# google-research/nerf-from-image

Measured on NVIDIA H100. Metric: rays_per_sec_128x128_64+64spp, higher is better.
Workload: dtype f32

## Files before the change

### nerf_from_image_b200/csrc/nfi_forward_pipe.cuh

```cuda
#pragma once
#include <type_traits>

#include "nfi_forward.cuh"
#include "nfi_forward_tc.cuh"

namespace nfi {

#ifndef NFI_WAIT_NS
#define NFI_WAIT_NS 0
#endif
#define NFI_STEP_WAIT(bar, par) tc::mbar_wait_backoff<NFI_WAIT_NS>(bar, par)

__device__ __forceinline__ void mbar_arrive(uint64_t* bar) {
  asm volatile("mbarrier.arrive.shared::cta.b64 _, [%0];" ::"r"(tc::smem_u32(bar)) : "memory");
}

__device__ __forceinline__ float ld_relaxed(const float* p) {
  float v;
  asm volatile("ld.relaxed.cta.global.f32 %0, [%1];" : "=f"(v) : "l"(p) : "memory");
  return v;
}

__device__ __forceinline__ bool elect_one() {
  uint32_t pred;
  asm volatile(
      "{\n.reg .pred p;\nelect.sync _|p, 0xffffffff;\nselp.u32 %0, 1, 0, p;\n}\n"
      : "=r"(pred));
  return pred != 0;
}

struct TileCoord {
  int b, tile_x, tile_y;
};

__device__ __forceinline__ TileCoord tile_coord(int tile, int tiles_x, int tiles_y) {
  TileCoord c;
  const int per_img = tiles_x * tiles_y;
  c.b = tile / per_img;
  const int r = tile % per_img;
  const int bx = (tiles_x + 1) / 2;
  const int blk = r / 4, in = r % 4;
  int tx = 2 * (blk % bx) + (in & 1), ty = 2 * (blk / bx) + (in >> 1);
  if ((tiles_x & 1) || (tiles_y & 1)) {
    tx = r % tiles_x;
    ty = r / tiles_x;
  }
  c.tile_x = tx;
  c.tile_y = ty;
  return c;
}

constexpr int kPipeSlots = 3;
constexpr int kPipeStageBytes = 32768;
constexpr int kFwdStageBytes = 16384;
constexpr int kD2Ld = 20;
constexpr int kD2SlotBytes = kThreads * kD2Ld * 4;

__host__ __device__ inline size_t pipe_scratch_floats(int S, int nes) {
  return tc_scratch_floats_per_group(S) + (size_t)S * kThreads * nes;
}

constexpr int kViewTileBytes = kThreads * NFI_VIEW_FEATURES * 4;

template <int P, bool VD = false>
struct PipeCfg {
  static constexpr int kThreadsTotal = 256 + 128 * P;
  static constexpr int kStages = P + 1;
  static constexpr int kSmA = VD ? 41984 : 25600;
  static constexpr int kSmD2 = kSmA + kStages * kFwdStageBytes;
  static constexpr int kSmView = kSmD2 + kPipeSlots * kD2SlotBytes;
  static constexpr int kSmPal = kSmView + (VD ? kViewTileBytes : 0);
  static constexpr int kSmFrac = kSmPal + 48 * 4;
  static constexpr int kSmBars = kSmFrac + 128 * 4;
  static constexpr int kNumBars = 2 * kStages + 2 * kPipeSlots + 3;
  static constexpr int kSmBytes = kSmBars + kNumBars * 8;
  static constexpr int kActRegs = 136;
  static constexpr int kShadeRegs = 80;
  static constexpr int kProducerRegs = 88;
};

constexpr float kLog2e = 1.4426950408889634f;
constexpr float kLn2 = 0.6931471805599453f;
constexpr float kPadLogit = -1e30f;

__device__ __forceinline__ void decoder_layer2(const float (&d)[32], uint64_t w2_hi, uint64_t w2_lo,
                                               const float* __restrict__ b1, float* d2, int warp,
                                               int lane) {
  uint32_t hi[8][4], lo[8][4];
  tc::softplus_frag<true>(d, b1, lane & 3, hi, lo);
  float o[8];
#pragma unroll
  for (int i = 0; i < 8; ++i) o[i] = 0.f;
  tc::wgmma_fence();
  tc::layer2_mb(o, hi, lo, w2_hi, w2_lo);
  tc::wgmma_commit();
  tc::wgmma_wait<0>();
  tc::reg_fence(o);
  tc::store_frag_rows(o, d2, kD2Ld, warp, lane);
}

template <typename F>
__device__ __forceinline__ void decoder_step(uint64_t dsc_a, uint64_t w1_hi, uint64_t w1_lo,
                                             uint64_t w2_hi, uint64_t w2_lo,
                                             const float* __restrict__ b1, float* d2, int warp,
                                             int lane, F&& on_stage_read) {
#pragma unroll 1
  for (int mb = 0; mb < 2; ++mb) {
    float d[32];
#pragma unroll
    for (int i = 0; i < 32; ++i) d[i] = 0.f;
    tc::wgmma_fence();
    tc::layer1_mb(d, dsc_a + mb * (8192 >> 4), dsc_a + ((16384 + mb * 8192) >> 4), w1_hi, w1_lo);
    tc::wgmma_commit();
    tc::wgmma_wait<0>();
    tc::reg_fence(d);
    if (mb == 1) on_stage_read();
    decoder_layer2(d, w2_hi, w2_lo, b1, d2 + 64 * mb * kD2Ld, warp, lane);
  }
}

template <typename F>
__device__ __forceinline__ void decoder_step_fp32(const unsigned char* stage, uint64_t w1_hi,
                                                  uint64_t w1_lo, uint64_t w2_hi, uint64_t w2_lo,
                                                  const float* __restrict__ b1, float* d2, int warp,
                                                  int lane, F&& on_stage_read) {
  float fa[4][4], fb[4][4];
  tc::load_afrag_sw128(fa, stage, 0, warp, lane);
  tc::load_afrag_sw128(fb, stage, 64, warp, lane);
  on_stage_read();
#pragma unroll 1
  for (int mb = 0; mb < 2; ++mb) {
    uint32_t a_hi[4][4], a_lo[4][4];
#pragma unroll
    for (int kb = 0; kb < 4; ++kb)
#pragma unroll
      for (int s = 0; s < 4; ++s) tc::put_split(a_hi, a_lo, kb, s, fa[kb][s]);
    float d[32];
#pragma unroll
    for (int i = 0; i < 32; ++i) d[i] = 0.f;
    tc::wgmma_fence();
    tc::layer1_mb_rs(d, a_hi, a_lo, w1_hi, w1_lo);
    tc::wgmma_commit();
    tc::wgmma_wait<0>();
    tc::reg_fence(d);
    decoder_layer2(d, w2_hi, w2_lo, b1, d2 + 64 * mb * kD2Ld, warp, lane);
#pragma unroll
    for (int kb = 0; kb < 4; ++kb)
#pragma unroll
      for (int s = 0; s < 4; ++s) fa[kb][s] = fb[kb][s];
  }
}

__device__ __forceinline__ void fill_view_tile(const nfi_render_params& p, const TileCoord& tcd,
                                               const float* __restrict__ b2f, float4* vt, int wig,
                                               int lane) {
  const int g = lane >> 2, t = lane & 3;
#pragma unroll
// ... 286 lines not shown
  const float* noise_t;
  const float* noise_u;
  const float* frac;
  int S, wig;
  bool explicit_noise;
};
template <int N>
__device__ __forceinline__ void resample_rows_impl(const ResampleArgs& a, int first, int count,
                                                   float tnear, float tfar, size_t ray, bool valid,
                                                   int lane) {
  const int S = a.S;
  if (count <= 0) return;
  struct In {
    LaneVec<N> w, n, u;
    size_t rayj;
  };
  auto load = [&](int j, In& in) {
    in.rayj = ((size_t)__shfl_sync(kFull, (unsigned)(ray >> 32), j) << 32) |
              (size_t)__shfl_sync(kFull, (unsigned)ray, j);
    const int col = 32 * a.wig + j;
#pragma unroll
    for (int i = 0; i < N; ++i) {
      const int e = 32 * i + lane;
      in.w.v[i] = (e < S) ? ldcg(a.sc_w + e * kThreads + col) : 0.f;
      in.n.v[i] = 0.f;
      if (a.explicit_noise) {
        in.n.v[i] = (e < S) ? a.noise_t[in.rayj * S + e] : 0.f;
        in.u.v[i] = (e < S) ? a.noise_u[in.rayj * S + e] : 2.f;
      } else {
        in.u.v[i] = (e < S) ? linspace01(e, S) : 2.f;
      }
    }
  };
  In cur, nxt;
  load(first, cur);
#pragma unroll 1
  for (int j = first; j < first + count; ++j) {
    load(j + 1 < first + count ? j + 1 : j, nxt);
    const float nearj = __shfl_sync(kFull, tnear, j), farj = __shfl_sync(kFull, tfar, j);
    const bool validj = __shfl_sync(kFull, (int)valid, j) != 0;
    const int col = 32 * a.wig + j;
    const float spanj = farj - nearj;
    LaneVec<N> t;
#pragma unroll
    for (int i = 0; i < N; ++i)
      t.v[i] = lerp_torch(nearj, farj, a.frac[32 * i + lane]) + cur.n.v[i] * (spanj / (float)S);
    const LaneVec<N> z = resample_ray<N>(cur.w, t, cur.u, !a.explicit_noise, S, lane);
#pragma unroll
    for (int i = 0; i < N; ++i) {
      const int e = 32 * i + lane;
      if (e < S) a.sc_zf[e * kThreads + col] = z.v[i];
      if (a.z_fine != nullptr && validj && e < S) a.z_fine[cur.rayj * S + e] = z.v[i];
    }
    cur = nxt;
  }
}
template <int NOUT_PAD, int EXTRA, bool FINE, int P, bool DBG, int NSLOT = 2, bool VD = false>
__global__ void __launch_bounds__(PipeCfg<P>::kThreadsTotal, 1)
render_forward_pipe(const nfi_render_params p, const unsigned char* __restrict__ wimg,
                    float* __restrict__ scratch) {
  using Cfg = PipeCfg<P, VD>;
  static_assert(!(VD && DBG), "the phase timers are not instantiated for the view-conditioned kernel");
  constexpr int kImgBytes = VD ? kVdBytes : kWiBytes;
  constexpr int kImgB1 = VD ? kVdB1 : kWiB1, kImgB2 = VD ? kVdHead : kWiB2;
  constexpr int NA_ = NOUT_PAD - 1;
  constexpr int NE = (EXTRA == 1) ? 3 : (EXTRA == 2 ? NA_ : 0);
  constexpr int NES = (EXTRA == 2) ? NA_ : 0;
  extern __shared__ __align__(1024) unsigned char smem_raw[];
  unsigned char* base = smem_raw;
  const int tid = threadIdx.x, lane = tid & 31;
  const int hw_wg = __shfl_sync(kFull, tid >> 7, 0);
  const int wg = (hw_wg < P) ? hw_wg + 3 : (P + 1 - hw_wg);
  const int gt = tid & 127;
  const int wig = __shfl_sync(kFull, gt >> 5, 0);
  const int S = p.num_samples;

  uint64_t* bars = reinterpret_cast<uint64_t*>(base + Cfg::kSmBars);
  constexpr int NS = Cfg::kStages;
  uint64_t* full = bars;
  uint64_t* a_free = full + NS;
  uint64_t* d2_full = a_free + NS;
  uint64_t* slot_free = d2_full + kPipeSlots;
  uint64_t* cw_ready = slot_free + kPipeSlots;
  uint64_t* zf_ready = cw_ready + 1;
  uint64_t* wbar = zf_ready + 1;
  float* d2s = reinterpret_cast<float*>(base + Cfg::kSmD2);
  const float* b1s = reinterpret_cast<const float*>(base + kImgB1);
  const float* b2s = reinterpret_cast<const float*>(base + kImgB2);
  float* pal = reinterpret_cast<float*>(base + Cfg::kSmPal);
  float* frac = reinterpret_cast<float*>(base + Cfg::kSmFrac);
  if (tid < 128) frac[tid] = (float)tid / (float)S;

  if (tid == 0) {
    if (tc::smem_u32(base) & 1023u) __trap();
    for (int i = 0; i < NS; ++i) {
      tc::mbar_init(&full[i], kWarps);
      tc::mbar_init(&a_free[i], kWarps);
    }
    for (int i = 0; i < kPipeSlots; ++i) {
      tc::mbar_init(&d2_full[i], kWarps);
      tc::mbar_init(&slot_free[i], kWarps);
    }
    tc::mbar_init(cw_ready, kWarps);
    tc::mbar_init(zf_ready, (2 + P) * kWarps);
    tc::mbar_init(wbar, 1);
    tc::fence_mbar_init();
  }
  __syncthreads();
  if (tid == 0) {
    tc::mbar_expect_tx(wbar, kImgBytes);
    tc::tma_bulk_g2s(base, wimg, kImgBytes, wbar);
  }
  tc::mbar_wait(wbar, 0);

  const int tiles_x = (p.width + kTileW - 1) / kTileW;
  const int tiles_y = (p.height + kTileH - 1) / kTileH;
  const int n_tiles = tiles_x * tiles_y * p.batch;
  const int my_tiles =
      ((int)blockIdx.x < n_tiles) ? (n_tiles - 1 - (int)blockIdx.x) / (int)gridDim.x + 1 : 0;
  const uint32_t total_steps = (uint32_t)my_tiles * (uint32_t)S * (FINE ? 2u : 1u);
  const int R = p.plane_res;
  const float inv_range = 1.f / p.scene_range;
  const bool explicit_noise = (p.noise_mode == NFI_NOISE_EXPLICIT);
  const bool dbg_skip_gather = (p.mlp_mode & 0x100) != 0;
  const bool dbg_skip_consumer = (p.mlp_mode & 0x200) != 0;
  const bool dbg_window = (p.mlp_mode & 0x800) != 0;
  const bool dbg_time = DBG && (p.mlp_mode & 0x1000) && p.normals != nullptr && blockIdx.x == 0 &&
                        lane == 0 && (wg <= 3) && wg != 2 && wig == 0;
  long long tacc[DBG ? 10 : 1];
  long long tprev = 0;
  if (DBG)
    for (int i = 0; i < 10; ++i) tacc[i] = 0;
#define NFI_T(i)                         \
  if (DBG && dbg_time) {                 \
    const long long now__ = clock64();   \
    tacc[i] += now__ - tprev;            \
    tprev = now__;                       \
  }
  float* slab = scratch + (size_t)blockIdx.x * pipe_scratch_floats(S, NES);
  float4* sc_srgb = reinterpret_cast<float4*>(slab);
  float* sc_t = slab + (size_t)4 * S * kThreads;
  float* sc_w = sc_t + (size_t)S * kThreads;
  float* sc_zf = sc_w + (size_t)S * kThreads;
  float* sc_e = sc_zf + (size_t)S * kThreads;

  constexpr int kRsParts = 2 + P;
  auto rs_first = [](int part) {
    constexpr int base_rows = 32 / kRsParts, rem = 32 % kRsParts;
    return part * base_rows + min(max(part - 2, 0), rem);
  };
  auto resample_rows = [&](int part, float tnear, float tfar, size_t ray, bool valid) {
    const int first = rs_first(part), count = rs_first(part + 1) - first;
    ResampleArgs ra;
    ra.sc_w = sc_w;
    ra.sc_zf = sc_zf;
    ra.z_fine = p.z_fine;
    ra.noise_t = p.noise_t;
    ra.noise_u = p.noise_u;
    ra.frac = frac;
    ra.S = S;
    ra.wig = wig;
    ra.explicit_noise = explicit_noise;
    resample_rows_impl<NSLOT>(ra, first, count, tnear, tfar, ray, valid, lane);
  };

  if (wg >= 3) {
    asm volatile("setmaxnreg.dec.sync.aligned.u32 %0;" ::"n"(Cfg::kProducerRegs));
    const int set = wg - 3;
    uint32_t n = 0;
    uint32_t tile_it = 0;
    for (int tile = blockIdx.x; tile < n_tiles; tile += gridDim.x, ++tile_it) {
      const TileCoord tcd = tile_coord(tile, tiles_x, tiles_y);
      const int b = tcd.b;
      int px, py;
      tile_pixel(tcd.tile_x, tcd.tile_y, wig, lane, px, py);
      const bool valid = (px < p.width) && (py < p.height);
      px = min(px, p.width - 1);
      py = min(py, p.height - 1);
      const size_t ray = ((size_t)b * p.height + py) * p.width + px;
      Ray r;
      setup_ray(p, b, py, px, r);
      const float span = r.tfar - r.tnear;
      const uint32_t plane_bytes = (uint32_t)R * (uint32_t)R * 128u;
      const unsigned char* planes_b =
          reinterpret_cast<const unsigned char*>(p.planes) + (size_t)b * 3 * plane_bytes;
      for (int pass = 0; pass < (FINE ? 2 : 1); ++pass) {
        if (pass == 1) {
          tc::mbar_wait(cw_ready, tile_it & 1);
          resample_rows(2 + set, r.tnear, r.tfar, ray, valid);
          __threadfence_block();
          __syncwarp();
          if (lane == 0) mbar_arrive(zf_ready);
          tc::mbar_wait(zf_ready, tile_it & 1);
        }
        int s = (int)(((uint32_t)set + (uint32_t)P - (n % P)) % P);
        auto fetch = [&](int ss) -> float {
          if (ss >= S) return 0.f;
          if (pass == 0) return explicit_noise ? p.noise_t[ray * S + ss] : 0.f;
          return ld_relaxed(sc_zf + ss * kThreads + gt);
        };
        float nxt = fetch(s);
        for (; s < S; s += P) {
          const uint32_t st = (n + (uint32_t)s) % NS, u = (n + (uint32_t)s) / NS;
          unsigned char* const stage = base + Cfg::kSmA + st * kFwdStageBytes;
          const float cur = nxt;
          nxt = fetch(s + P);
          if (DBG && dbg_time) tprev = clock64();
          NFI_STEP_WAIT(&a_free[st], (u & 1) ^ 1);
          NFI_T(0)
          float t;
          if (pass == 0)
            t = lerp_torch(r.tnear, r.tfar, frac[s]) + cur * (span / (float)S);
          else
            t = cur;
          const float x0 = (r.ox + r.dx * t) * inv_range, x1 = (r.oy + r.dy * t) * inv_range,
                      x2 = (r.oz + r.dz * t) * inv_range;
          ByteTaps tp;
          byte_taps(x0, x1, R, 0u, tp.o[0], tp.fx[0], tp.fy[0]);
          byte_taps(x0, x2, R, plane_bytes >> 4, tp.o[1], tp.fx[1], tp.fy[1]);
          byte_taps(x1, x2, R, plane_bytes >> 3, tp.o[2], tp.fx[2], tp.fy[2]);
          NFI_T(1)
          if (dbg_window) {
            tp.o[0] &= 0x7FFu;
            tp.o[1] &= 0x7FFu;
            tp.o[2] &= 0x7FFu;
          }
          if (!dbg_skip_gather)
            gather_to_tiles_lean<TileStore::kFp32>(planes_b, R, tp, stage, nullptr, 32 * wig, lane);
          NFI_T(2)
          __syncwarp();
          if (lane == 0) mbar_arrive(&full[st]);
          NFI_T(3)
          if (DBG && dbg_time) tacc[9] += 1;
        }
        n += (uint32_t)S;
      }
    }
    if (DBG && dbg_time)
      for (int i = 0; i < 10; ++i) p.normals[i] = (float)tacc[i];
  } else if (wg == 0) {
    asm volatile("setmaxnreg.inc.sync.aligned.u32 %0;" ::"n"(Cfg::kActRegs));
    const uint32_t base_s = tc::smem_u32(base);
    const uint64_t dsc_w1_hi = tc::gmma_desc_sw128(base_s + kWiW1Hi);
    const uint64_t dsc_w1_lo = tc::gmma_desc_sw128(base_s + kWiW1Lo);
    const uint64_t dsc_w2_hi = tc::gmma_desc_sw128(base_s + (VD ? kVdW2Hi : kWiW2Hi));
    const uint64_t dsc_w2_lo = tc::gmma_desc_sw128(base_s + (VD ? kVdW2Lo : kWiW2Lo));
    const float4* vt = reinterpret_cast<const float4*>(base + Cfg::kSmView) + gt;
    uint32_t st = 0, u = 0, sl = 0, v = 0;
    auto activate = [&]() {
      if (DBG && dbg_time && tprev == 0) tprev = clock64();
      NFI_T(2)
      NFI_STEP_WAIT(&full[st], u & 1);
      NFI_STEP_WAIT(&slot_free[sl], (v & 1) ^ 1);
      NFI_T(0)
      float* d2 = d2s + sl * (kThreads * kD2Ld);
      if constexpr (VD) {
        decoder_step_vd(base + Cfg::kSmA + st * kFwdStageBytes, dsc_w1_hi, dsc_w1_lo, dsc_w2_hi,
                        dsc_w2_lo, tc::gmma_desc_sw128(base_s + kVdW3Hi),
                        tc::gmma_desc_sw128(base_s + kVdW3Lo), b1s, vt, d2, wig, lane, [&]() {
                          __syncwarp();
                          if (lane == 0) mbar_arrive(&a_free[st]);
                        });
      } else if (!dbg_skip_consumer) {
        decoder_step_fp32(base + Cfg::kSmA + st * kFwdStageBytes, dsc_w1_hi, dsc_w1_lo, dsc_w2_hi,
                          dsc_w2_lo, b1s, d2, wig, lane, [&]() {
                            __syncwarp();
                            if (lane == 0) mbar_arrive(&a_free[st]);
                          });
      } else {
        __syncwarp();
        if (lane == 0) mbar_arrive(&a_free[st]);
      }
      __syncwarp();
      if (lane == 0) mbar_arrive(&d2_full[sl]);
      if (++st == NS) { st = 0; ++u; }
      if (++sl == kPipeSlots) { sl = 0; ++v; }
      NFI_T(1)
      if (DBG && dbg_time) tacc[9] += 1;
    };
    uint32_t tile_it = 0;
    for (int tile = blockIdx.x; tile < n_tiles; tile += gridDim.x, ++tile_it) {
      if constexpr (VD)
        fill_view_tile(p, tile_coord(tile, tiles_x, tiles_y),
                       reinterpret_cast<const float*>(base + kVdB2f),
                       reinterpret_cast<float4*>(base + Cfg::kSmView) + gt, wig, lane);
      for (int s = 0; s < S; ++s) activate();
      if (FINE) {
        const TileCoord tcd = tile_coord(tile, tiles_x, tiles_y);
        int px, py;
        tile_pixel(tcd.tile_x, tcd.tile_y, wig, lane, px, py);
        const bool valid = (px < p.width) && (py < p.height);
        px = min(px, p.width - 1);
        py = min(py, p.height - 1);
        const size_t ray = ((size_t)tcd.b * p.height + py) * p.width + px;
        Ray r;
        setup_ray(p, tcd.b, py, px, r);
        tc::mbar_wait(cw_ready, tile_it & 1);
        NFI_T(3)
        resample_rows(1, r.tnear, r.tfar, ray, valid);
        __threadfence_block();
        __syncwarp();
        if (lane == 0) mbar_arrive(zf_ready);
        NFI_T(4)
        for (int s = 0; s < S; ++s) activate();
      }
    }
    if (DBG && dbg_time)
      for (int i = 0; i < 10; ++i) p.normals[16 + i] = (float)tacc[i];
  } else {
    asm volatile("setmaxnreg.dec.sync.aligned.u32 %0;" ::"n"(Cfg::kShadeRegs));
    uint32_t sl = 0, v = 0;
    FieldConst fc;
    fc.A = p.n_attention;
    fc.use_sdf = p.use_sdf;
    fc.inv_beta = p.use_sdf ? 1.f / p.beta[0] : 0.f;
    fc.inv_alpha = p.use_sdf ? 1.f / p.alpha[0] : 0.f;

    uint32_t tile_it = 0;
    for (int tile = blockIdx.x; tile < n_tiles; tile += gridDim.x, ++tile_it) {
      const TileCoord tcd = tile_coord(tile, tiles_x, tiles_y);
      const int b = tcd.b;
      int px, py;
      tile_pixel(tcd.tile_x, tcd.tile_y, wig, lane, px, py);
      const bool valid = (px < p.width) && (py < p.height);
      px = min(px, p.width - 1);
      py = min(py, p.height - 1);
      const size_t ray = ((size_t)b * p.height + py) * p.width + px;
      Ray r;
      setup_ray(p, b, py, px, r);
      const float span = r.tfar - r.tnear;

      tc::bar_sync(1, kThreads);
      if (gt < 48)
        pal[gt] = (p.n_attention > 0 && gt < p.n_attention * 3)
                      ? p.palette[(size_t)b * p.n_attention * 3 + gt]
                      : 0.f;
      tc::bar_sync(1, kThreads);
      Compositor<NE, true> comp;
      comp.init();

      auto shade = [&](float t, float& sigma, float& cr, float& cg, float& cb, float* ex) {
        const float* d2 = d2s + sl * (kThreads * kD2Ld) + gt * kD2Ld;
        if (DBG && dbg_time && tprev == 0) tprev = clock64();
        NFI_T(2)
        NFI_STEP_WAIT(&d2_full[sl], v & 1);
        NFI_T(0)
        float o16[16];
#pragma unroll
        for (int o4 = 0; o4 < 4; ++o4) {
          const float4 x = *reinterpret_cast<const float4*>(d2 + 4 * o4);
          o16[4 * o4] = x.x;
          o16[4 * o4 + 1] = x.y;
          o16[4 * o4 + 2] = x.z;
          o16[4 * o4 + 3] = x.w;
        }
        __syncwarp();
        if (lane == 0) mbar_arrive(&slot_free[sl]);
        if (++sl == kPipeSlots) { sl = 0; ++v; }
        const float wx = r.ox + r.dx * t, wy = r.oy + r.dy * t, wz = r.oz + r.dz * t;
        const float x0 = wx * inv_range, x1 = wy * inv_range, x2 = wz * inv_range;
        const float keep =
            (fabsf(x0) > 1.f || fabsf(x1) > 1.f || fabsf(x2) > 1.f) ? 0.f : 1.f;
        float out[NOUT_PAD];
#pragma unroll
        for (int o4 = 0; o4 < NOUT_PAD / 4; ++o4) {
          const float4 bb = *reinterpret_cast<const float4*>(b2s + 4 * o4);
          out[4 * o4] = o16[4 * o4] + bb.x;
          out[4 * o4 + 1] = o16[4 * o4 + 1] + bb.y;
          out[4 * o4 + 2] = o16[4 * o4 + 2] + bb.z;
          out[4 * o4 + 3] = o16[4 * o4 + 3] + bb.w;
        }
        if (dbg_skip_consumer) {
          sigma = out[0];
          cr = cg = cb = out[1];
        } else {
          field_head_fast<NOUT_PAD>(out, fc, pal, keep, sigma, cr, cg, cb,
                                    EXTRA == 2 ? ex : nullptr);
        }
        if (EXTRA == 1) {
          ex[0] = wx;
          ex[1] = wy;
          ex[2] = wz;
        }
        NFI_T(1)
        if (DBG && dbg_time) tacc[9] += 1;
      };

      {
        float wT = 1.f, prev_t = 0.f, prev_s = 0.f;
        const float4* nz4 = reinterpret_cast<const float4*>(p.noise_t + ray * S);
        const float4 zero4 = make_float4(0.f, 0.f, 0.f, 0.f);
        float4 nzc = explicit_noise ? nz4[0] : zero4;
        float4 nzn = (explicit_noise && S > 4) ? nz4[1] : zero4;
        const float jit = span / (float)S;
        for (int s = 0; s < S; ++s) {
          const int sq = s & 3;
          const float nz = sq == 0 ? nzc.x : (sq == 1 ? nzc.y : (sq == 2 ? nzc.z : nzc.w));
          const float t = lerp_torch(r.tnear, r.tfar, frac[s]) + nz * jit;
          if (sq == 3) {
            nzc = nzn;
            nzn = (explicit_noise && s + 5 < S) ? nz4[(s + 5) >> 2] : zero4;
          }
          float sigma, cr, cg, cb;
          float ex[NE > 0 ? NE : 1];
          shade(t, sigma, cr, cg, cb, ex);
          if (FINE) {
            sc_srgb[s * kThreads + gt] = make_float4(sigma, cr, cg, cb);
            sc_t[s * kThreads + gt] = t;
#pragma unroll
            for (int a = 0; a < NES; ++a) sc_e[((size_t)s * NES + a) * kThreads + gt] = ex[a];
            if (s > 0) {
              const float delta = (t - prev_t) * r.dn;
              const float a = 1.f - __expf(-prev_s * delta);
              sc_w[(s - 1) * kThreads + gt] = a * wT;
              wT = wT * ((1.f - a) + 1e-10f);
            }
            prev_t = t;
            prev_s = sigma;
          } else {
            comp.push(t, sigma, cr, cg, cb, ex, r.dn);
          }
          NFI_T(3)
        }
      }

      if (FINE) {
        sc_w[(S - 1) * kThreads + gt] = 0.f;
        __threadfence_block();
        __syncwarp();
        if (lane == 0) mbar_arrive(cw_ready);
        tc::mbar_wait(cw_ready, tile_it & 1);
        NFI_T(4)
        resample_rows(0, r.tnear, r.tfar, ray, valid);
        __threadfence_block();
        __syncwarp();
        if (lane == 0) mbar_arrive(zf_ready);
        tc::mbar_wait(zf_ready, tile_it & 1);
        NFI_T(5)

        int c = 0;
        float ct0 = ldcg(sc_t + gt), ct1 = ldcg(sc_t + kThreads + gt);
        float4 cq0 = __ldcg(sc_srgb + gt), cq1 = __ldcg(sc_srgb + kThreads + gt);
        auto take_coarse = [&]() {
          float ce[NE > 0 ? NE : 1];
          if (EXTRA == 1) {
            ce[0] = r.ox + r.dx * ct0;
            ce[1] = r.oy + r.dy * ct0;
            ce[2] = r.oz + r.dz * ct0;
          }
#pragma unroll
          for (int a = 0; a < NES; ++a) ce[a] = ldcg(sc_e + ((size_t)c * NES + a) * kThreads + gt);
          comp.push(ct0, cq0.x, cq0.y, cq0.z, cq0.w, ce, r.dn);
          ++c;
          ct0 = ct1;
          cq0 = cq1;
          if (c + 1 < S) {
            ct1 = ldcg(sc_t + (c + 1) * kThreads + gt);
            cq1 = __ldcg(sc_srgb + (c + 1) * kThreads + gt);
          }
        };
        float z0 = ldcg(sc_zf + gt);
        float z1 = (S > 1) ? ldcg(sc_zf + kThreads + gt) : 0.f;
        for (int k = 0; k < S; ++k) {
          const float z = z0;
          z0 = z1;
          z1 = (k + 2 < S) ? ldcg(sc_zf + (k + 2) * kThreads + gt) : 0.f;
          float sigma, cr, cg, cb;
          float ex[NE > 0 ? NE : 1];
          shade(z, sigma, cr, cg, cb, ex);
          while (c < S && ct0 <= z) take_coarse();
          comp.push(z, sigma, cr, cg, cb, ex, r.dn);
          NFI_T(3)
        }
        while (c < S) take_coarse();
        NFI_T(6)
      }

      if (valid) {
        float bg = 0.f;
        if (p.white_background) bg = 1.f - comp.am;
        p.rgb[ray * 3 + 0] = comp.ar + bg;
        p.rgb[ray * 3 + 1] = comp.ag + bg;
        p.rgb[ray * 3 + 2] = comp.ab + bg;
        p.depth[ray] = comp.ad;
        p.mask[ray] = comp.am;
        for (int q = 0; q < p.n_peers; ++q) {
          float* pr = p.peer_rgb[q] + ray * 3;
          pr[0] = comp.ar + bg;
          pr[1] = comp.ag + bg;
          pr[2] = comp.ab + bg;
          p.peer_depth[q][ray] = comp.ad;
          p.peer_mask[q][ray] = comp.am;
        }
        if (EXTRA == 1 && p.extra != nullptr)
          for (int a = 0; a < 3; ++a) p.extra[ray * 3 + a] = comp.ae[a];
        if (EXTRA == 2 && p.extra != nullptr)
          for (int a = 0; a < NE; ++a)
            if (a < p.n_attention) p.extra[ray * p.n_attention + a] = comp.ae[a];
      }
    }
    if (DBG && dbg_time)
      for (int i = 0; i < 10; ++i) p.normals[32 + i] = (float)tacc[i];
  }
#undef NFI_T
  __syncthreads();
  if (p.n_peers > 0 && p.peer_done != nullptr && tid == 0) {
    __threadfence_system();
    const unsigned done = atomicAdd(p.peer_done, 1u);
    if (done == gridDim.x - 1) {
      __threadfence();
      *p.peer_done = 0u;
      for (int q = 0; q < p.n_peers; ++q)
        asm volatile("st.release.sys.global.u32 [%0], %1;" ::"l"(p.peer_signal[q]), "r"(p.peer_epoch)
                     : "memory");
      const long long t0 = clock64();
      for (int q = 0; q < p.n_peers; ++q) {
        const uint32_t* flag = p.peer_signal_self + p.peer_rank[q];
        uint32_t v;
        do {
          asm volatile("ld.acquire.sys.global.u32 %0, [%1];" : "=r"(v) : "l"(flag) : "memory");
          if ((int)(v - p.peer_epoch) >= 0) break;
          __nanosleep(200);
          if (clock64() - t0 > 60000000000LL) __trap();
        } while (true);
      }
    }
  }
}

}
```

Before: 35.97 million.

## Software-pipeline coarse and fine passes across tiles with double-buffered scratch

```diff
diff --git a/nerf_from_image_b200/csrc/nfi_forward_pipe.cuh b/nerf_from_image_b200/csrc/nfi_forward_pipe.cuh
--- a/nerf_from_image_b200/csrc/nfi_forward_pipe.cuh
+++ b/nerf_from_image_b200/csrc/nfi_forward_pipe.cuh
@@ -13,6 +13,17 @@
 
 __device__ __forceinline__ void mbar_arrive(uint64_t* bar) {
   asm volatile("mbarrier.arrive.shared::cta.b64 _, [%0];" ::"r"(tc::smem_u32(bar)) : "memory");
+}
+
+__device__ __forceinline__ bool mbar_test_wait(uint64_t* bar, uint32_t parity) {
+  uint32_t ok;
+  asm volatile(
+      "{\n.reg .pred p;\nmbarrier.test_wait.parity.shared::cta.b64 p, [%1], %2;\n"
+      "selp.u32 %0, 1, 0, p;\n}\n"
+      : "=r"(ok)
+      : "r"(tc::smem_u32(bar)), "r"(parity)
+      : "memory");
+  return ok != 0;
 }
 
 __device__ __forceinline__ float ld_relaxed(const float* p) {
@@ -56,8 +67,11 @@
 constexpr int kD2Ld = 20;
 constexpr int kD2SlotBytes = kThreads * kD2Ld * 4;
 
+__host__ __device__ inline size_t pipe_scratch_slot_floats(int S, int nes) {
+  return tc_scratch_floats_per_group(S) + (size_t)S * kThreads * nes;
+}
 __host__ __device__ inline size_t pipe_scratch_floats(int S, int nes) {
-  return tc_scratch_floats_per_group(S) + (size_t)S * kThreads * nes;
+  return 2 * pipe_scratch_slot_floats(S, nes);
 }
 
 constexpr int kViewTileBytes = kThreads * NFI_VIEW_FEATURES * 4;
@@ -70,9 +84,9 @@
   static constexpr int kSmD2 = kSmA + kStages * kFwdStageBytes;
   static constexpr int kSmView = kSmD2 + kPipeSlots * kD2SlotBytes;
   static constexpr int kSmPal = kSmView + (VD ? kViewTileBytes : 0);
-  static constexpr int kSmFrac = kSmPal + 48 * 4;
+  static constexpr int kSmFrac = kSmPal + 2 * 48 * 4;
   static constexpr int kSmBars = kSmFrac + 128 * 4;
-  static constexpr int kNumBars = 2 * kStages + 2 * kPipeSlots + 3;
+  static constexpr int kNumBars = 2 * kStages + 2 * kPipeSlots + 5;
   static constexpr int kSmBytes = kSmBars + kNumBars * 8;
   static constexpr int kActRegs = 136;
   static constexpr int kShadeRegs = 80;
@@ -525,8 +539,8 @@
   uint64_t* d2_full = a_free + NS;
   uint64_t* slot_free = d2_full + kPipeSlots;
   uint64_t* cw_ready = slot_free + kPipeSlots;
-  uint64_t* zf_ready = cw_ready + 1;
-  uint64_t* wbar = zf_ready + 1;
+  uint64_t* zf_ready = cw_ready + 2;
+  uint64_t* wbar = zf_ready + 2;
   float* d2s = reinterpret_cast<float*>(base + Cfg::kSmD2);
   const float* b1s = reinterpret_cast<const float*>(base + kImgB1);
   const float* b2s = reinterpret_cast<const float*>(base + kImgB2);
@@ -544,8 +558,10 @@
       tc::mbar_init(&d2_full[i], kWarps);
       tc::mbar_init(&slot_free[i], kWarps);
     }
-    tc::mbar_init(cw_ready, kWarps);
-    tc::mbar_init(zf_ready, (2 + P) * kWarps);
+    for (int i = 0; i < 2; ++i) {
+      tc::mbar_init(&cw_ready[i], kWarps);
+      tc::mbar_init(&zf_ready[i], P * kWarps);
+    }
     tc::mbar_init(wbar, 1);
     tc::fence_mbar_init();
   }
@@ -561,7 +577,6 @@
   const int n_tiles = tiles_x * tiles_y * p.batch;
   const int my_tiles =
       ((int)blockIdx.x < n_tiles) ? (n_tiles - 1 - (int)blockIdx.x) / (int)gridDim.x + 1 : 0;
-  const uint32_t total_steps = (uint32_t)my_tiles * (uint32_t)S * (FINE ? 2u : 1u);
   const int R = p.plane_res;
   const float inv_range = 1.f / p.scene_range;
   const bool explicit_noise = (p.noise_mode == NFI_NOISE_EXPLICIT);
@@ -570,33 +585,64 @@
   const bool dbg_window = (p.mlp_mode & 0x800) != 0;
   const bool dbg_time = DBG && (p.mlp_mode & 0x1000) && p.normals != nullptr && blockIdx.x == 0 &&
                         lane == 0 && (wg <= 3) && wg != 2 && wig == 0;
-  long long tacc[DBG ? 10 : 1];
+  constexpr int kNT = DBG ? 12 : 1;
+  long long tacc[kNT];
   long long tprev = 0;
   if (DBG)
-    for (int i = 0; i < 10; ++i) tacc[i] = 0;
+    for (int i = 0; i < kNT; ++i) tacc[i] = 0;
 #define NFI_T(i)                         \
   if (DBG && dbg_time) {                 \
     const long long now__ = clock64();   \
     tacc[i] += now__ - tprev;            \
     tprev = now__;                       \
   }
-  float* slab = scratch + (size_t)blockIdx.x * pipe_scratch_floats(S, NES);
-  float4* sc_srgb = reinterpret_cast<float4*>(slab);
-  float* sc_t = slab + (size_t)4 * S * kThreads;
-  float* sc_w = sc_t + (size_t)S * kThreads;
-  float* sc_zf = sc_w + (size_t)S * kThreads;
-  float* sc_e = sc_zf + (size_t)S * kThreads;
-
-  constexpr int kRsParts = 2 + P;
-  auto rs_first = [](int part) {
-    constexpr int base_rows = 32 / kRsParts, rem = 32 % kRsParts;
-    return part * base_rows + min(max(part - 2, 0), rem);
+  struct Slot {
+    float4* srgb;
+    float* t;
+    float* w;
+    float* zf;
+    float* e;
   };
-  auto resample_rows = [&](int part, float tnear, float tfar, size_t ray, bool valid) {
-    const int first = rs_first(part), count = rs_first(part + 1) - first;
+  auto slot_of = [&](int k) {
+    float* slab = scratch + (size_t)blockIdx.x * pipe_scratch_floats(S, NES) +
+                  (size_t)(k & 1) * pipe_scratch_slot_floats(S, NES);
+    Slot o;
+    o.srgb = reinterpret_cast<float4*>(slab);
+    o.t = slab + (size_t)4 * S * kThreads;
+    o.w = o.t + (size_t)S * kThreads;
+    o.zf = o.w + (size_t)S * kThreads;
+    o.e = o.zf + (size_t)S * kThreads;
+    return o;
+  };
+  struct RowRay {
+    int b;
+    bool valid;
+    size_t ray;
+    Ray r;
+  };
+  auto row_ray = [&](int k) {
+    const TileCoord tcd = tile_coord((int)blockIdx.x + k * (int)gridDim.x, tiles_x, tiles_y);
+    int px, py;
+    tile_pixel(tcd.tile_x, tcd.tile_y, wig, lane, px, py);
+    RowRay o;
+    o.b = tcd.b;
+    o.valid = (px < p.width) && (py < p.height);
+    px = min(px, p.width - 1);
+    py = min(py, p.height - 1);
+    o.ray = ((size_t)tcd.b * p.height + py) * p.width + px;
+    setup_ray(p, tcd.b, py, px, o.r);
+    return o;
+  };
+
+  auto rs_first = [](int set) {
+    constexpr int base_rows = 32 / P, rem = 32 % P;
+    return set * base_rows + min(set, rem);
+  };
+  auto resample_rows = [&](int k, int first, int count, const RowRay& rr) {
+    const Slot sc = slot_of(k);
     ResampleArgs ra;
-    ra.sc_w = sc_w;
-    ra.sc_zf = sc_zf;
+    ra.sc_w = sc.w;
+    ra.sc_zf = sc.zf;
     ra.z_fine = p.z_fine;
     ra.noise_t = p.noise_t;
     ra.noise_u = p.noise_u;
@@ -604,83 +650,109 @@
     ra.S = S;
     ra.wig = wig;
     ra.explicit_noise = explicit_noise;
-    resample_rows_impl<NSLOT>(ra, first, count, tnear, tfar, ray, valid, lane);
+    resample_rows_impl<NSLOT>(ra, first, count, rr.r.tnear, rr.r.tfar, rr.ray, rr.valid, lane);
   };
 
   if (wg >= 3) {
     asm volatile("setmaxnreg.dec.sync.aligned.u32 %0;" ::"n"(Cfg::kProducerRegs));
     const int set = wg - 3;
+    const int rs0 = rs_first(set), rs_n = rs_first(set + 1) - rs0;
     uint32_t n = 0;
-    uint32_t tile_it = 0;
-    for (int tile = blockIdx.x; tile < n_tiles; tile += gridDim.x, ++tile_it) {
-      const TileCoord tcd = tile_coord(tile, tiles_x, tiles_y);
-      const int b = tcd.b;
-      int px, py;
-      tile_pixel(tcd.tile_x, tcd.tile_y, wig, lane, px, py);
-      const bool valid = (px < p.width) && (py < p.height);
-      px = min(px, p.width - 1);
-      py = min(py, p.height - 1);
-      const size_t ray = ((size_t)b * p.height + py) * p.width + px;
-      Ray r;
-      setup_ray(p, b, py, px, r);
+    auto resample_rest = [&](int k, int done, const RowRay& rq) {
+      if (done < rs_n) {
+        tc::mbar_wait(&cw_ready[k & 1], (k >> 1) & 1);
+        resample_rows(k, rs0 + done, rs_n - done, rq);
+      }
+      __threadfence_block();
+      __syncwarp();
+      if (lane == 0) mbar_arrive(&zf_ready[k & 1]);
+    };
+    auto run_pass = [&](int k, bool fine_pass, int rs) {
+      const RowRay rr = row_ray(k);
+      const Slot sc = slot_of(k);
+      const Ray& r = rr.r;
       const float span = r.tfar - r.tnear;
       const uint32_t plane_bytes = (uint32_t)R * (uint32_t)R * 128u;
       const unsigned char* planes_b =
-          reinterpret_cast<const unsigned char*>(p.planes) + (size_t)b * 3 * plane_bytes;
-      for (int pass = 0; pass < (FINE ? 2 : 1); ++pass) {
-        if (pass == 1) {
-          tc::mbar_wait(cw_ready, tile_it & 1);
-          resample_rows(2 + set, r.tnear, r.tfar, ray, valid);
-          __threadfence_block();
-          __syncwarp();
-          if (lane == 0) mbar_arrive(zf_ready);
-          tc::mbar_wait(zf_ready, tile_it & 1);
+          reinterpret_cast<const unsigned char*>(p.planes) + (size_t)rr.b * 3 * plane_bytes;
+      if (fine_pass) {
+        if (DBG && dbg_time) tprev = clock64();
+        tc::mbar_wait(&zf_ready[k & 1], (k >> 1) & 1);
+        NFI_T(5)
+      }
+      RowRay rq;
+      if (rs >= 0) rq = row_ray(rs);
+      int s = (int)(((uint32_t)set + (uint32_t)P - (n % P)) % P);
+      const int n_own = (S - s + P - 1) / P;
+      int j = 0, done = 0;
+      bool cw_seen = false;
+      auto fetch = [&](int ss) -> float {
+        if (ss >= S) return 0.f;
+        if (!fine_pass) return explicit_noise ? p.noise_t[rr.ray * S + ss] : 0.f;
+        return ld_relaxed(sc.zf + ss * kThreads + gt);
+      };
+      float nxt = fetch(s);
+      for (; s < S; s += P, ++j) {
+        const uint32_t st = (n + (uint32_t)s) % NS, u = (n + (uint32_t)s) / NS;
+        unsigned char* const stage = base + Cfg::kSmA + st * kFwdStageBytes;
+        const float cur = nxt;
+        nxt = fetch(s + P);
+        if (DBG && dbg_time) tprev = clock64();
+        NFI_STEP_WAIT(&a_free[st], (u & 1) ^ 1);
+        NFI_T(0)
+        float t;
+        if (!fine_pass)
+          t = lerp_torch(r.tnear, r.tfar, frac[s]) + cur * (span / (float)S);
+        else
+          t = cur;
+        const float x0 = (r.ox + r.dx * t) * inv_range, x1 = (r.oy + r.dy * t) * inv_range,
+                    x2 = (r.oz + r.dz * t) * inv_range;
+        ByteTaps tp;
+        byte_taps(x0, x1, R, 0u, tp.o[0], tp.fx[0], tp.fy[0]);
+        byte_taps(x0, x2, R, plane_bytes >> 4, tp.o[1], tp.fx[1], tp.fy[1]);
+        byte_taps(x1, x2, R, plane_bytes >> 3, tp.o[2], tp.fx[2], tp.fy[2]);
+        NFI_T(1)
+        if (dbg_window) {
+          tp.o[0] &= 0x7FFu;
+          tp.o[1] &= 0x7FFu;
+          tp.o[2] &= 0x7FFu;
         }
-        int s = (int)(((uint32_t)set + (uint32_t)P - (n % P)) % P);
-        auto fetch = [&](int ss) -> float {
-          if (ss >= S) return 0.f;
-          if (pass == 0) return explicit_noise ? p.noise_t[ray * S + ss] : 0.f;
-          return ld_relaxed(sc_zf + ss * kThreads + gt);
-        };
-        float nxt = fetch(s);
-        for (; s < S; s += P) {
-          const uint32_t st = (n + (uint32_t)s) % NS, u = (n + (uint32_t)s) / NS;
-          unsigned char* const stage = base + Cfg::kSmA + st * kFwdStageBytes;
-          const float cur = nxt;
-          nxt = fetch(s + P);
+        if (!dbg_skip_gather)
+          gather_to_tiles_lean<TileStore::kFp32>(planes_b, R, tp, stage, nullptr, 32 * wig, lane);
+        NFI_T(2)
+        __syncwarp();
+        if (lane == 0) mbar_arrive(&full[st]);
+        NFI_T(3)
+        if (rs >= 0) {
+          const int upto = (rs_n * (j + 1) + n_own - 1) / n_own;
+          if (upto > done && !cw_seen)
+            cw_seen = __all_sync(kFull, mbar_test_wait(&cw_ready[rs & 1], (rs >> 1) & 1));
+          if (upto > done && cw_seen) {
+            resample_rows(rs, rs0 + done, upto - done, rq);
+            done = upto;
+          }
+          NFI_T(4)
+        }
+        if (DBG && dbg_time) tacc[9] += 1;
+      }
+      n += (uint32_t)S;
+      if (rs >= 0) resample_rest(rs, done, rq);
+    };
+    for (int k = 0; k <= my_tiles; ++k) {
+      if (k < my_tiles) run_pass(k, false, (FINE && k >= 1) ? k - 1 : -1);
+      if (FINE && k >= 1) {
+        if (k == my_tiles) {
           if (DBG && dbg_time) tprev = clock64();
-          NFI_STEP_WAIT(&a_free[st], (u & 1) ^ 1);
-          NFI_T(0)
-          float t;
-          if (pass == 0)
-            t = lerp_torch(r.tnear, r.tfar, frac[s]) + cur * (span / (float)S);
-          else
-            t = cur;
-          const float x0 = (r.ox + r.dx * t) * inv_range, x1 = (r.oy + r.dy * t) * inv_range,
-                      x2 = (r.oz + r.dz * t) * inv_range;
-          ByteTaps tp;
-          byte_taps(x0, x1, R, 0u, tp.o[0], tp.fx[0], tp.fy[0]);
-          byte_taps(x0, x2, R, plane_bytes >> 4, tp.o[1], tp.fx[1], tp.fy[1]);
-          byte_taps(x1, x2, R, plane_bytes >> 3, tp.o[2], tp.fx[2], tp.fy[2]);
-          NFI_T(1)
-          if (dbg_window) {
-            tp.o[0] &= 0x7FFu;
-            tp.o[1] &= 0x7FFu;
-            tp.o[2] &= 0x7FFu;
-          }
-          if (!dbg_skip_gather)
-            gather_to_tiles_lean<TileStore::kFp32>(planes_b, R, tp, stage, nullptr, 32 * wig, lane);
-          NFI_T(2)
-          __syncwarp();
-          if (lane == 0) mbar_arrive(&full[st]);
-          NFI_T(3)
-          if (DBG && dbg_time) tacc[9] += 1;
+          resample_rest(k - 1, 0, row_ray(k - 1));
+          NFI_T(4)
         }
-        n += (uint32_t)S;
-      }
-    }
-    if (DBG && dbg_time)
-      for (int i = 0; i < 10; ++i) p.normals[i] = (float)tacc[i];
+        run_pass(k - 1, true, -1);
+      }
+    }
+    if (DBG && dbg_time) {
+      tacc[11] = (long long)my_tiles;
+      for (int i = 0; i < kNT; ++i) p.normals[i] = (float)tacc[i];
+    }
   } else if (wg == 0) {
     asm volatile("setmaxnreg.inc.sync.aligned.u32 %0;" ::"n"(Cfg::kActRegs));
     const uint32_t base_s = tc::smem_u32(base);
@@ -690,12 +762,23 @@
     const uint64_t dsc_w2_lo = tc::gmma_desc_sw128(base_s + (VD ? kVdW2Lo : kWiW2Lo));
     const float4* vt = reinterpret_cast<const float4*>(base + Cfg::kSmView) + gt;
     uint32_t st = 0, u = 0, sl = 0, v = 0;
-    auto activate = [&]() {
+    long long tend = 0;
+    auto activate = [&](int s, bool fine_pass) {
       if (DBG && dbg_time && tprev == 0) tprev = clock64();
       NFI_T(2)
       NFI_STEP_WAIT(&full[st], u & 1);
+      if (s < NS) {
+        NFI_T(4)
+      } else {
+        NFI_T(0)
+      }
+      if (DBG && dbg_time && fine_pass && s == 0) tacc[8] += tprev - tend;
       NFI_STEP_WAIT(&slot_free[sl], (v & 1) ^ 1);
-      NFI_T(0)
+      if (s < NS) {
+        NFI_T(5)
+      } else {
+        NFI_T(3)
+      }
       float* d2 = d2s + sl * (kThreads * kD2Ld);
       if constexpr (VD) {
         decoder_step_vd(base + Cfg::kSmA + st * kFwdStageBytes, dsc_w1_hi, dsc_w1_lo, dsc_w2_hi,
@@ -719,37 +802,27 @@
       if (++st == NS) { st = 0; ++u; }
       if (++sl == kPipeSlots) { sl = 0; ++v; }
       NFI_T(1)
-      if (DBG && dbg_time) tacc[9] += 1;
+      if (DBG && dbg_time) {
+        tacc[9] += 1;
+        tend = tprev;
+      }
     };
-    uint32_t tile_it = 0;
-    for (int tile = blockIdx.x; tile < n_tiles; tile += gridDim.x, ++tile_it) {
+    auto run_pass = [&](int k, bool fine_pass) {
       if constexpr (VD)
-        fill_view_tile(p, tile_coord(tile, tiles_x, tiles_y),
+        fill_view_tile(p, tile_coord((int)blockIdx.x + k * (int)gridDim.x, tiles_x, tiles_y),
                        reinterpret_cast<const float*>(base + kVdB2f),
                        reinterpret_cast<float4*>(base + Cfg::kSmView) + gt, wig, lane);
-      for (int s = 0; s < S; ++s) activate();
-      if (FINE) {
-        const TileCoord tcd = tile_coord(tile, tiles_x, tiles_y);
-        int px, py;
-        tile_pixel(tcd.tile_x, tcd.tile_y, wig, lane, px, py);
-        const bool valid = (px < p.width) && (py < p.height);
-        px = min(px, p.width - 1);
-        py = min(py, p.height - 1);
-        const size_t ray = ((size_t)tcd.b * p.height + py) * p.width + px;
-        Ray r;
-        setup_ray(p, tcd.b, py, px, r);
-        tc::mbar_wait(cw_ready, tile_it & 1);
-        NFI_T(3)
-        resample_rows(1, r.tnear, r.tfar, ray, valid);
-        __threadfence_block();
-        __syncwarp();
-        if (lane == 0) mbar_arrive(zf_ready);
-        NFI_T(4)
-        for (int s = 0; s < S; ++s) activate();
-      }
-    }
-    if (DBG && dbg_time)
-      for (int i = 0; i < 10; ++i) p.normals[16 + i] = (float)tacc[i];
+      for (int s = 0; s < S; ++s) activate(s, fine_pass);
+    };
+    for (int k = 0; k <= my_tiles; ++k) {
+      if (k < my_tiles) run_pass(k, false);
+      if (FINE && k >= 1) run_pass(k - 1, true);
+    }
+    if (DBG && dbg_time) {
+      NFI_T(10)
+      tacc[11] = (long long)my_tiles;
+      for (int i = 0; i < kNT; ++i) p.normals[16 + i] = (float)tacc[i];
+    }
   } else {
     asm volatile("setmaxnreg.dec.sync.aligned.u32 %0;" ::"n"(Cfg::kShadeRegs));
     uint32_t sl = 0, v = 0;
@@ -759,191 +832,195 @@
     fc.inv_beta = p.use_sdf ? 1.f / p.beta[0] : 0.f;
     fc.inv_alpha = p.use_sdf ? 1.f / p.alpha[0] : 0.f;
 
-    uint32_t tile_it = 0;
-    for (int tile = blockIdx.x; tile < n_tiles; tile += gridDim.x, ++tile_it) {
-      const TileCoord tcd = tile_coord(tile, tiles_x, tiles_y);
-      const int b = tcd.b;
-      int px, py;
-      tile_pixel(tcd.tile_x, tcd.tile_y, wig, lane, px, py);
-      const bool valid = (px < p.width) && (py < p.height);
-      px = min(px, p.width - 1);
-      py = min(py, p.height - 1);
-      const size_t ray = ((size_t)b * p.height + py) * p.width + px;
-      Ray r;
-      setup_ray(p, b, py, px, r);
-      const float span = r.tfar - r.tnear;
-
+    auto shade = [&](const Ray& r, const float* palk, float t, float& sigma, float& cr, float& cg,
+                     float& cb, float* ex) {
+      const float* d2 = d2s + sl * (kThreads * kD2Ld) + gt * kD2Ld;
+      if (DBG && dbg_time && tprev == 0) tprev = clock64();
+      NFI_T(2)
+      NFI_STEP_WAIT(&d2_full[sl], v & 1);
+      NFI_T(0)
+      float o16[16];
+#pragma unroll
+      for (int o4 = 0; o4 < 4; ++o4) {
+        const float4 x = *reinterpret_cast<const float4*>(d2 + 4 * o4);
+        o16[4 * o4] = x.x;
+        o16[4 * o4 + 1] = x.y;
+        o16[4 * o4 + 2] = x.z;
+        o16[4 * o4 + 3] = x.w;
+      }
+      __syncwarp();
+      if (lane == 0) mbar_arrive(&slot_free[sl]);
+      if (++sl == kPipeSlots) { sl = 0; ++v; }
+      const float wx = r.ox + r.dx * t, wy = r.oy + r.dy * t, wz = r.oz + r.dz * t;
+      const float x0 = wx * inv_range, x1 = wy * inv_range, x2 = wz * inv_range;
+      const float keep =
+          (fabsf(x0) > 1.f || fabsf(x1) > 1.f || fabsf(x2) > 1.f) ? 0.f : 1.f;
+      float out[NOUT_PAD];
+#pragma unroll
+      for (int o4 = 0; o4 < NOUT_PAD / 4; ++o4) {
+        const float4 bb = *reinterpret_cast<const float4*>(b2s + 4 * o4);
+        out[4 * o4] = o16[4 * o4] + bb.x;
+        out[4 * o4 + 1] = o16[4 * o4 + 1] + bb.y;
+        out[4 * o4 + 2] = o16[4 * o4 + 2] + bb.z;
+        out[4 * o4 + 3] = o16[4 * o4 + 3] + bb.w;
+      }
+      if (dbg_skip_consumer) {
+        sigma = out[0];
+        cr = cg = cb = out[1];
+      } else {
+        field_head_fast<NOUT_PAD>(out, fc, palk, keep, sigma, cr, cg, cb,
+                                  EXTRA == 2 ? ex : nullptr);
+      }
+      if (EXTRA == 1) {
+        ex[0] = wx;
+        ex[1] = wy;
+        ex[2] = wz;
+      }
+      NFI_T(1)
+      if (DBG && dbg_time) tacc[9] += 1;
+    };
+
+    auto write_out = [&](const RowRay& rr, const Compositor<NE, true>& comp) {
+      if (!rr.valid) return;
+      const size_t ray = rr.ray;
+      float bg = 0.f;
+      if (p.white_background) bg = 1.f - comp.am;
+      p.rgb[ray * 3 + 0] = comp.ar + bg;
+      p.rgb[ray * 3 + 1] = comp.ag + bg;
+      p.rgb[ray * 3 + 2] = comp.ab + bg;
+      p.depth[ray] = comp.ad;
+      p.mask[ray] = comp.am;
+      for (int q = 0; q < p.n_peers; ++q) {
+        float* pr = p.peer_rgb[q] + ray * 3;
+        pr[0] = comp.ar + bg;
+        pr[1] = comp.ag + bg;
+        pr[2] = comp.ab + bg;
+        p.peer_depth[q][ray] = comp.ad;
+        p.peer_mask[q][ray] = comp.am;
+      }
+      if (EXTRA == 1 && p.extra != nullptr)
+        for (int a = 0; a < 3; ++a) p.extra[ray * 3 + a] = comp.ae[a];
+      if (EXTRA == 2 && p.extra != nullptr)
+        for (int a = 0; a < NE; ++a)
+          if (a < p.n_attention) p.extra[ray * p.n_attention + a] = comp.ae[a];
+    };
+
+    auto coarse_pass = [&](int k) {
+      const RowRay rr = row_ray(k);
+      const Ray& r = rr.r;
+      const Slot sc = slot_of(k);
+      float* palk = pal + 48 * (k & 1);
       tc::bar_sync(1, kThreads);
       if (gt < 48)
-        pal[gt] = (p.n_attention > 0 && gt < p.n_attention * 3)
-                      ? p.palette[(size_t)b * p.n_attention * 3 + gt]
-                      : 0.f;
+        palk[gt] = (p.n_attention > 0 && gt < p.n_attention * 3)
+                       ? p.palette[(size_t)rr.b * p.n_attention * 3 + gt]
+                       : 0.f;
       tc::bar_sync(1, kThreads);
       Compositor<NE, true> comp;
       comp.init();
-
-      auto shade = [&](float t, float& sigma, float& cr, float& cg, float& cb, float* ex) {
-        const float* d2 = d2s + sl * (kThreads * kD2Ld) + gt * kD2Ld;
-        if (DBG && dbg_time && tprev == 0) tprev = clock64();
-        NFI_T(2)
-        NFI_STEP_WAIT(&d2_full[sl], v & 1);
-        NFI_T(0)
-        float o16[16];
-#pragma unroll
-        for (int o4 = 0; o4 < 4; ++o4) {
-          const float4 x = *reinterpret_cast<const float4*>(d2 + 4 * o4);
-          o16[4 * o4] = x.x;
-          o16[4 * o4 + 1] = x.y;
-          o16[4 * o4 + 2] = x.z;
-          o16[4 * o4 + 3] = x.w;
+      const float span = r.tfar - r.tnear;
+      float wT = 1.f, prev_t = 0.f, prev_s = 0.f;
+      const float4* nz4 = reinterpret_cast<const float4*>(p.noise_t + rr.ray * S);
+      const float4 zero4 = make_float4(0.f, 0.f, 0.f, 0.f);
+      float4 nzc = explicit_noise ? nz4[0] : zero4;
+      float4 nzn = (explicit_noise && S > 4) ? nz4[1] : zero4;
+      const float jit = span / (float)S;
+      for (int s = 0; s < S; ++s) {
+        const int sq = s & 3;
+        const float nz = sq == 0 ? nzc.x : (sq == 1 ? nzc.y : (sq == 2 ? nzc.z : nzc.w));
+        const float t = lerp_torch(r.tnear, r.tfar, frac[s]) + nz * jit;
+        if (sq == 3) {
+          nzc = nzn;
+          nzn = (explicit_noise && s + 5 < S) ? nz4[(s + 5) >> 2] : zero4;
         }
-        __syncwarp();
-        if (lane == 0) mbar_arrive(&slot_free[sl]);
-        if (++sl == kPipeSlots) { sl = 0; ++v; }
-        const float wx = r.ox + r.dx * t, wy = r.oy + r.dy * t, wz = r.oz + r.dz * t;
-        const float x0 = wx * inv_range, x1 = wy * inv_range, x2 = wz * inv_range;
-        const float keep =
-            (fabsf(x0) > 1.f || fabsf(x1) > 1.f || fabsf(x2) > 1.f) ? 0.f : 1.f;
-        float out[NOUT_PAD];
-#pragma unroll
-        for (int o4 = 0; o4 < NOUT_PAD / 4; ++o4) {
-          const float4 bb = *reinterpret_cast<const float4*>(b2s + 4 * o4);
-          out[4 * o4] = o16[4 * o4] + bb.x;
-          out[4 * o4 + 1] = o16[4 * o4 + 1] + bb.y;
-          out[4 * o4 + 2] = o16[4 * o4 + 2] + bb.z;
-          out[4 * o4 + 3] = o16[4 * o4 + 3] + bb.w;
+        float sigma, cr, cg, cb;
+        float ex[NE > 0 ? NE : 1];
+        shade(r, palk, t, sigma, cr, cg, cb, ex);
+        if (FINE) {
+          sc.srgb[s * kThreads + gt] = make_float4(sigma, cr, cg, cb);
+          sc.t[s * kThreads + gt] = t;
+#pragma unroll
+          for (int a = 0; a < NES; ++a) sc.e[((size_t)s * NES + a) * kThreads + gt] = ex[a];
+          if (s > 0) {
+            const float delta = (t - prev_t) * r.dn;
+            const float a = 1.f - __expf(-prev_s * delta);
+            sc.w[(s - 1) * kThreads + gt] = a * wT;
+            wT = wT * ((1.f - a) + 1e-10f);
+          }
+          prev_t = t;
+          prev_s = sigma;
+        } else {
+          comp.push(t, sigma, cr, cg, cb, ex, r.dn);
         }
-        if (dbg_skip_consumer) {
-          sigma = out[0];
-          cr = cg = cb = out[1];
-        } else {
-          field_head_fast<NOUT_PAD>(out, fc, pal, keep, sigma, cr, cg, cb,
-                                    EXTRA == 2 ? ex : nullptr);
-        }
-        if (EXTRA == 1) {
-          ex[0] = wx;
-          ex[1] = wy;
-          ex[2] = wz;
-        }
-        NFI_T(1)
-        if (DBG && dbg_time) tacc[9] += 1;
-      };
-
-      {
-        float wT = 1.f, prev_t = 0.f, prev_s = 0.f;
-        const float4* nz4 = reinterpret_cast<const float4*>(p.noise_t + ray * S);
-        const float4 zero4 = make_float4(0.f, 0.f, 0.f, 0.f);
-        float4 nzc = explicit_noise ? nz4[0] : zero4;
-        float4 nzn = (explicit_noise && S > 4) ? nz4[1] : zero4;
-        const float jit = span / (float)S;
-        for (int s = 0; s < S; ++s) {
-          const int sq = s & 3;
-          const float nz = sq == 0 ? nzc.x : (sq == 1 ? nzc.y : (sq == 2 ? nzc.z : nzc.w));
-          const float t = lerp_torch(r.tnear, r.tfar, frac[s]) + nz * jit;
-          if (sq == 3) {
-            nzc = nzn;
-            nzn = (explicit_noise && s + 5 < S) ? nz4[(s + 5) >> 2] : zero4;
-          }
-          float sigma, cr, cg, cb;
-          float ex[NE > 0 ? NE : 1];
-          shade(t, sigma, cr, cg, cb, ex);
-          if (FINE) {
-            sc_srgb[s * kThreads + gt] = make_float4(sigma, cr, cg, cb);
-            sc_t[s * kThreads + gt] = t;
-#pragma unroll
-            for (int a = 0; a < NES; ++a) sc_e[((size_t)s * NES + a) * kThreads + gt] = ex[a];
-            if (s > 0) {
-              const float delta = (t - prev_t) * r.dn;
-              const float a = 1.f - __expf(-prev_s * delta);
-              sc_w[(s - 1) * kThreads + gt] = a * wT;
-              wT = wT * ((1.f - a) + 1e-10f);
-            }
-            prev_t = t;
-            prev_s = sigma;
-          } else {
-            comp.push(t, sigma, cr, cg, cb, ex, r.dn);
-          }
-          NFI_T(3)
-        }
-      }
-
+        NFI_T(3)
+      }
       if (FINE) {
-        sc_w[(S - 1) * kThreads + gt] = 0.f;
+        sc.w[(S - 1) * kThreads + gt] = 0.f;
         __threadfence_block();
         __syncwarp();
-        if (lane == 0) mbar_arrive(cw_ready);
-        tc::mbar_wait(cw_ready, tile_it & 1);
-        NFI_T(4)
-        resample_rows(0, r.tnear, r.tfar, ray, valid);
-        __threadfence_block();
-        __syncwarp();
-        if (lane == 0) mbar_arrive(zf_ready);
-        tc::mbar_wait(zf_ready, tile_it & 1);
-        NFI_T(5)
-
-        int c = 0;
-        float ct0 = ldcg(sc_t + gt), ct1 = ldcg(sc_t + kThreads + gt);
-        float4 cq0 = __ldcg(sc_srgb + gt), cq1 = __ldcg(sc_srgb + kThreads + gt);
-        auto take_coarse = [&]() {
-          float ce[NE > 0 ? NE : 1];
-          if (EXTRA == 1) {
-            ce[0] = r.ox + r.dx * ct0;
-            ce[1] = r.oy + r.dy * ct0;
-            ce[2] = r.oz + r.dz * ct0;
-          }
-#pragma unroll
-          for (int a = 0; a < NES; ++a) ce[a] = ldcg(sc_e + ((size_t)c * NES + a) * kThreads + gt);
-          comp.push(ct0, cq0.x, cq0.y, cq0.z, cq0.w, ce, r.dn);
-          ++c;
-          ct0 = ct1;
-          cq0 = cq1;
-          if (c + 1 < S) {
-            ct1 = ldcg(sc_t + (c + 1) * kThreads + gt);
-            cq1 = __ldcg(sc_srgb + (c + 1) * kThreads + gt);
-          }
-        };
-        float z0 = ldcg(sc_zf + gt);
-        float z1 = (S > 1) ? ldcg(sc_zf + kThreads + gt) : 0.f;
-        for (int k = 0; k < S; ++k) {
-          const float z = z0;
-          z0 = z1;
-          z1 = (k + 2 < S) ? ldcg(sc_zf + (k + 2) * kThreads + gt) : 0.f;
-          float sigma, cr, cg, cb;
-          float ex[NE > 0 ? NE : 1];
-          shade(z, sigma, cr, cg, cb, ex);
-          while (c < S && ct0 <= z) take_coarse();
-          comp.push(z, sigma, cr, cg, cb, ex, r.dn);
-          NFI_T(3)
+        if (lane == 0) mbar_arrive(&cw_ready[k & 1]);
+      } else {
+        write_out(rr, comp);
+      }
+    };
+
+    auto fine_pass = [&](int k) {
+      const RowRay rr = row_ray(k);
+      const Ray& r = rr.r;
+      const Slot sc = slot_of(k);
+      const float* palk = pal + 48 * (k & 1);
+      if (DBG && dbg_time) tprev = clock64();
+      tc::mbar_wait(&zf_ready[k & 1], (k >> 1) & 1);
+      NFI_T(5)
+      Compositor<NE, true> comp;
+      comp.init();
+      int c = 0;
+      float ct0 = ldcg(sc.t + gt), ct1 = ldcg(sc.t + kThreads + gt);
+      float4 cq0 = __ldcg(sc.srgb + gt), cq1 = __ldcg(sc.srgb + kThreads + gt);
+      auto take_coarse = [&]() {
+        float ce[NE > 0 ? NE : 1];
+        if (EXTRA == 1) {
+          ce[0] = r.ox + r.dx * ct0;
+          ce[1] = r.oy + r.dy * ct0;
+          ce[2] = r.oz + r.dz * ct0;
         }
-        while (c < S) take_coarse();
-        NFI_T(6)
-      }
-
-      if (valid) {
-        float bg = 0.f;
-        if (p.white_background) bg = 1.f - comp.am;
-        p.rgb[ray * 3 + 0] = comp.ar + bg;
-        p.rgb[ray * 3 + 1] = comp.ag + bg;
-        p.rgb[ray * 3 + 2] = comp.ab + bg;
-        p.depth[ray] = comp.ad;
-        p.mask[ray] = comp.am;
-        for (int q = 0; q < p.n_peers; ++q) {
-          float* pr = p.peer_rgb[q] + ray * 3;
-          pr[0] = comp.ar + bg;
-          pr[1] = comp.ag + bg;
-          pr[2] = comp.ab + bg;
-          p.peer_depth[q][ray] = comp.ad;
-          p.peer_mask[q][ray] = comp.am;
+#pragma unroll
+        for (int a = 0; a < NES; ++a) ce[a] = ldcg(sc.e + ((size_t)c * NES + a) * kThreads + gt);
+        comp.push(ct0, cq0.x, cq0.y, cq0.z, cq0.w, ce, r.dn);
+        ++c;
+        ct0 = ct1;
+        cq0 = cq1;
+        if (c + 1 < S) {
+          ct1 = ldcg(sc.t + (c + 1) * kThreads + gt);
+          cq1 = __ldcg(sc.srgb + (c + 1) * kThreads + gt);
         }
-        if (EXTRA == 1 && p.extra != nullptr)
-          for (int a = 0; a < 3; ++a) p.extra[ray * 3 + a] = comp.ae[a];
-        if (EXTRA == 2 && p.extra != nullptr)
-          for (int a = 0; a < NE; ++a)
-            if (a < p.n_attention) p.extra[ray * p.n_attention + a] = comp.ae[a];
-      }
-    }
-    if (DBG && dbg_time)
-      for (int i = 0; i < 10; ++i) p.normals[32 + i] = (float)tacc[i];
+      };
+      float z0 = ldcg(sc.zf + gt);
+      float z1 = (S > 1) ? ldcg(sc.zf + kThreads + gt) : 0.f;
+      for (int k2 = 0; k2 < S; ++k2) {
+        const float z = z0;
+        z0 = z1;
+        z1 = (k2 + 2 < S) ? ldcg(sc.zf + (k2 + 2) * kThreads + gt) : 0.f;
+        float sigma, cr, cg, cb;
+        float ex[NE > 0 ? NE : 1];
+        shade(r, palk, z, sigma, cr, cg, cb, ex);
+        while (c < S && ct0 <= z) take_coarse();
+        comp.push(z, sigma, cr, cg, cb, ex, r.dn);
+        NFI_T(3)
+      }
+      while (c < S) take_coarse();
+      NFI_T(6)
+      write_out(rr, comp);
+    };
+
+    for (int k = 0; k <= my_tiles; ++k) {
+      if (k < my_tiles) coarse_pass(k);
+      if (FINE && k >= 1) fine_pass(k - 1);
+    }
+    if (DBG && dbg_time) {
+      tacc[11] = (long long)my_tiles;
+      for (int i = 0; i < kNT; ++i) p.normals[32 + i] = (float)tacc[i];
+    }
   }
 #undef NFI_T
   __syncthreads();
```

After: 35.82 million, median of 6. Within noise of the previous version (-0.4%).
